# OliBus801/TARL-simulator

Measured on AMD Instinct MI355X. Metric: ppo_env_steps_per_sec, higher is better.
Workload: dtype f32; 1 GPU; mpnn+ppo train, 10000-edge torus dual graph, 16384 agents, T=256 (BASELINE config 4); envs_per_gpu=32768, parallelism=dp1, rollout_kernels=frames

## Files before the change

### tarl-simulator_amd/csrc/fused.hip

```cpp
#include "fused_common.h"

struct PlanOut {
  const int32_t* out_ptr;
  const int32_t* out_dst;
};

__global__ __launch_bounds__(FB) void k_pack_nodes(const float* __restrict__ x, Layout L, int64_t B, int64_t N,
                                                   const float* __restrict__ cong, FusedBufs fb, float4* st0_out,
                                                   PlanOut P) {
  const int64_t gid = (int64_t)blockIdx.x * FB + threadIdx.x;
  if (gid >= B * N) return;
  const int64_t i = gid / B;
  const int64_t b = gid - i * B;
  const float* xi = x + b * L.bstride + i * L.ldx;
  const int Nmax = L.Nmax;
  const float n = xi[L.col_n()];
  const int q = (int)n;
  const float tail = (q >= 1 && q <= Nmax) ? xi[q - 1] : 0.0f;
  const float head = xi[0];
  if (q < 0 || q > 127 || !(head >= 0.0f && head < 16777216.0f) || !(tail >= 0.0f && tail < 16777216.0f))
    atomicOr(fb.flags, FLAG_PACK_RANGE);
  bool dirty = q >= Nmax - 1;
  for (int sidx = q < 0 ? 0 : q; sidx < Nmax; ++sidx)
    dirty = dirty || xi[sidx] != 0.0f || xi[Nmax + sidx] != 0.0f || xi[2 * Nmax + sidx] != 0.0f;
// ... 941 lines not shown
  RowStat rs[NCH];
#pragma unroll
  for (int r = 0; r < NCH; ++r) {
    const NodeRec& nr = nodes[ri[r]];
    rs[r] = RowStat{nr.out_deg, nr.out0, nr.tt0, nr.maxn};
  }
  if (threadIdx.x == 0) s_cnt = 0;
  __syncthreads();
  float nsum = 0.0f;
  if (valid) {
    uint32_t pa[NCH], tlw[NCH], pj[NCH][4];
    uint2 hp[NCH];
    uint32_t ovf = 0u;
#pragma unroll
    for (int r = 0; r < NCH; ++r) {
      const uint32_t row = (uint32_t)ri[r] * B + b;
      pa[r] = at32<O32>(post, row);
      if (SIB) {
        if (r == 0) {
          const int32_t* od = rchunks[blockIdx.y].out4;
#pragma unroll
          for (int q = 0; q < 4; ++q) pj[0][q] = at32<O32>(post, (uint32_t)od[q] * B + b);
        } else {
#pragma unroll
          for (int q = 0; q < 4; ++q) pj[r][q] = pj[0][q];
        }
      } else {
        const int32_t* od = nodes[ri[r]].out4;
#pragma unroll
        for (int q = 0; q < 4; ++q) pj[r][q] = at32<O32>(post, (uint32_t)od[q] * B + b);
      }
    }
#pragma unroll
    for (int r = 0; r < NCH; ++r) {
      const uint32_t row = (uint32_t)ri[r] * B + b;
      hp[r] = make_uint2(0u, 0u);
      tlw[r] = 0u;
      if (Nmax < 2 || (pa[r] & (PF_ARRIVED | PF_NONEMPTY | PF_TLAUTH))) {
        hp[r] = at32<O32>(fb.hdp, row);
        tlw[r] = at32<O32>(fb.tl, row);
      }
    }
#pragma unroll
    for (int r = 0; r < NCH; ++r)
      if (live[r]) {
        bool pop;
        float n = 0.0f;
        const uint32_t i = (uint32_t)ri[r];
        const bool ev = row_phase_a<FAPI, O32>(i, b, rs[r], post, pa[r], hp[r], tlw[r], pj[r], Nmax, B, N, fb, A, t, out, &pop, &n);
        nsum += n;
        if (ev) {
          const int32_t pos = atomicAdd(&s_cnt, 1);
          if (pos < EV_CAP) {
            s_item[pos] = (uint16_t)((r << 9) | (pop ? 256 : 0) | threadIdx.x);
            s_words[pos] = make_uint4(pa[r], hp[r].x, hp[r].y, tlw[r]);
          } else {
            ovf |= (1u << r) | (pop ? (16u << r) : 0u);
          }
        }
      }
    if (ovf != 0u) {
#pragma unroll 1
      for (int r = 0; r < NCH; ++r) {
        if (!((ovf >> r) & 1u)) continue;
        uint32_t pa_r = pa[0], tl_r = tlw[0];
        uint2 hp_r = hp[0];
        int32_t i_r = ri[0];
#pragma unroll
        for (int q = 1; q < NCH; ++q) {
          pa_r = (r == q) ? pa[q] : pa_r;
          tl_r = (r == q) ? tlw[q] : tl_r;
          hp_r.x = (r == q) ? hp[q].x : hp_r.x;
          hp_r.y = (r == q) ? hp[q].y : hp_r.y;
          i_r = (r == q) ? ri[q] : i_r;
        }
        const float2 nc = row_phase_b<FAPI>((uint32_t)i_r, b, ((ovf >> (4 + r)) & 1u) != 0u, pa_r, hp_r, tl_r, nodes[i_r], out_ptr,
                                      out_dst, Nmax, B, N, fb, ag, A, a_bstride, t, out);
        nsum -= nc.y;
        if (nc.y != 0.0f) atomicAdd(&fb.acc_w[(int64_t)(blockIdx.y % (unsigned)fb.acc_slots) * B + b], nc.y);
      }
    }
  }
  const int64_t bank0 = (int64_t)(blockIdx.y % (unsigned)fb.acc_slots) * B;
  if (valid && nsum != 0.0f) atomicAdd(&fb.acc_n[bank0 + b], nsum);
  __syncthreads();
  const int32_t cnt = s_cnt < EV_CAP ? s_cnt : EV_CAP;
  for (int32_t idx = threadIdx.x; idx < cnt; idx += blockDim.x) {
    const uint32_t item = s_item[idx];
    const uint32_t r = item >> 9, lane2 = item & 255u;
    const uint4 wd = s_words[idx];
    const uint32_t b2 = blockIdx.x * blockDim.x + lane2;
    int32_t i2 = ri[0];
#pragma unroll
    for (int q = 1; q < NCH; ++q) i2 = (r == (uint32_t)q) ? ri[q] : i2;
    const float2 nc = row_phase_b<FAPI>((uint32_t)i2, b2, (item & 256u) != 0u, wd.x, make_uint2(wd.y, wd.z), wd.w, nodes[i2],
                                  out_ptr, out_dst, Nmax, B, N, fb, ag, A, a_bstride, t, out);
    if (nc.y != 0.0f) {
      atomicAdd(&fb.acc_n[bank0 + b2], -nc.y);
      atomicAdd(&fb.acc_w[bank0 + b2], nc.y);
    }
  }
}

__device__ __forceinline__ bool fused_target(const FusedBufs& fb, PlanOut P, const uint8_t* __restrict__ sel8, int64_t b,
                                             int64_t B, int64_t N, int32_t origin, int32_t* road, int32_t* cap) {
  if (origin < 0 || origin >= N) return false;
  const int64_t orow = (int64_t)origin * B + b;
  const uint32_t c = sel8[orow] & 0x7Fu;
  const long long r = (long long)(c == SEL_RAW ? fb.sel[orow] : (float)P.out_dst[P.out_ptr[origin] + (int32_t)c]);
  if (r < 0 || r >= N) return false;
  const long long room = (long long)(fb.st0[r].x - TARL_CONGESTION_FILE - (float)(fb.hdp[r * B + b].x & HD_CNT));
  *road = (int32_t)r;
  *cap = (int32_t)(room > 0x7fffffff ? 0x7fffffff : room);
  return room > 0;
}

__device__ __forceinline__ bool fused_target_words(const FusedBufs& fb, PlanOut P, const uint8_t* __restrict__ sel8,
                                                   int64_t b, int64_t B, int64_t N, int32_t origin, int32_t* road,
                                                   uint32_t* hd_out, uint32_t* tl_out) {
  if (origin < 0 || origin >= N) return false;
  const int64_t orow = (int64_t)origin * B + b;
  const uint32_t c = sel8[orow] & 0x7Fu;
  const int32_t* o4 = fb.nodes[origin].out4;
  const int32_t t0 = o4[0], t1 = o4[1], t2 = o4[2], t3 = o4[3];
  long long r;
  if (c < 4u)
    r = (long long)(float)(c == 0u ? t0 : (c == 1u ? t1 : (c == 2u ? t2 : t3)));
  else
    r = (long long)(c == SEL_RAW ? fb.sel[orow] : (float)P.out_dst[P.out_ptr[origin] + (int32_t)c]);
  if (r < 0 || r >= N) return false;
  const uint32_t hd = fb.hdp[r * B + b].x;
  *tl_out = fb.tl[r * B + b];
  const long long room = (long long)(fb.st0[r].x - TARL_CONGESTION_FILE - (float)(hd & HD_CNT));
  *road = (int32_t)r;
  *hd_out = hd;
  return room > 0;
}

struct InsLds {
  int32_t wave[INSB / 64];
  int32_t cnt, adm, lo;
  int32_t cnt2[8], adm2[8], lo2[8];
  int32_t un_agent[INS_CAP], un_road[INS_CAP], un_k[INS_CAP];
  uint32_t un_hd[INS_CAP], un_tl[INS_CAP];
};
#define s_wave L.wave
#define s_cnt L.cnt
#define s_adm L.adm
#define s_lo L.lo
#define s_un_agent L.un_agent
#define s_un_road L.un_road
#define s_un_k L.un_k
#define s_un_hd L.un_hd
#define s_un_tl L.un_tl
__device__ __forceinline__ void fused_insert_body(InsLds& L, int64_t b, int Nmax, int64_t B, int64_t N, const FusedBufs& fb, PlanOut P,
                                                  const uint8_t* __restrict__ sel8, float* __restrict__ ag, int64_t A,
                                                  int64_t a_bstride, int use_cong, float t,
                                                  int32_t* __restrict__ scratch, const float* __restrict__ entropy_in,
                                                  float* __restrict__ reward, FrameOut out,
                                                  float* __restrict__ log_prob, float* __restrict__ entropy) {
  float* agb = ag + b * a_bstride;
  int32_t* cand_agent = scratch + b * 2 * A;
  int32_t* cand_road = cand_agent + A;
  const int tid = threadIdx.x, lane = tid & 63, wid = tid >> 6;

  if (tid == 0) {
    s_cnt = 0;
    s_adm = 0;
  }
  long long lpf = 0;
  float nf = 0.0f, wf = 0.0f;
  if (wid == 0) {
    for (int64_t sl_ = lane; sl_ < fb.acc_slots; sl_ += 64) {
      lpf += fb.acc_lp[sl_ * B + b];
      nf += fb.acc_n[sl_ * B + b];
      wf += fb.acc_w[sl_ * B + b];
      fb.acc_lp[sl_ * B + b] = 0;
      fb.acc_n[sl_ * B + b] = 0.0f;
      fb.acc_w[sl_ * B + b] = 0.0f;
    }
  }
  __syncthreads();
  if (fb.a_order) {
    const int32_t* ord = fb.a_order + b * A;
    const float* dsort = fb.a_dep_sorted + b * A;
    const int32_t lo = fb.cur_lo[b];
    if (tid == 0) s_lo = 0x7fffffff;
    __syncthreads();
    for (int64_t k0 = lo; k0 < A; k0 += INSB) {
      const int64_t k = k0 + tid;
      bool notdue = false;
      if (k < A) {
        bool due, waiting;
        int32_t a, origin;
        if (fb.a_win) {
          const uint4 w = fb.a_win[b * A + k];
          waiting = fb.a_ins[b * A + k] == 0;
          due = __uint_as_float(w.x) <= t;
          origin = (int32_t)w.y;
          a = (int32_t)w.z;
        } else {
          due = dsort[k] <= t;
          a = due ? ord[k] : 0;
          waiting = due && fb.a_status[b * A + a] == 0;
          origin = waiting ? fb.a_origin[b * A + a] : 0;
        }
        notdue = !due;
        if (!due) {
          atomicMin(&s_lo, (int32_t)k);
        } else if (waiting) {
          atomicMin(&s_lo, (int32_t)k);
          int32_t road = 0, cap = 0;
          if (fb.a_win) {
            uint32_t hdw = 0u, tlw = 0u;
            if (fused_target_words(fb, P, sel8, b, B, N, origin, &road, &hdw, &tlw)) {
              const int32_t pos = atomicAdd(&s_cnt, 1);
              if (pos < INS_CAP) {
                s_un_agent[pos] = a;
                s_un_road[pos] = road;
                s_un_k[pos] = (int32_t)k;
                s_un_hd[pos] = hdw;
                s_un_tl[pos] = tlw;
              }
            }
          } else if (fused_target(fb, P, sel8, b, B, N, origin, &road, &cap)) {
            const int32_t pos = atomicAdd(&s_cnt, 1);
            if (pos < INS_CAP) {
              s_un_agent[pos] = a;
              s_un_road[pos] = road;
            }
          }
        }
      }
      if (__syncthreads_or(notdue ? 1 : 0)) break;
    }
    __syncthreads();
    if (tid == 0) fb.cur_lo[b] = s_lo == 0x7fffffff ? (int32_t)A : s_lo;
  } else {
    for (int64_t a0 = tid; a0 < A; a0 += 4 * INSB) {
      uint8_t stt[4];
      float dp[4];
  #pragma unroll
      for (int j = 0; j < 4; ++j) {
        const int64_t a = a0 + (int64_t)j * INSB;
        stt[j] = a < A ? fb.a_status[b * A + a] : (uint8_t)1;
        dp[j] = a < A ? fb.a_dep[b * A + a] : 0.0f;
      }
  #pragma unroll
      for (int j = 0; j < 4; ++j) {
        if (stt[j] == 0 && dp[j] <= t) {
          const int64_t a = a0 + (int64_t)j * INSB;
          int32_t road = 0, cap = 0;
          if (fused_target(fb, P, sel8, b, B, N, fb.a_origin[b * A + a], &road, &cap)) {
            const int32_t pos = atomicAdd(&s_cnt, 1);
            if (pos < INS_CAP) {
              s_un_agent[pos] = (int32_t)a;
              s_un_road[pos] = road;
            }
          }
        }
      }
// ... 66 lines not shown
      if (a < A && fb.a_status[b * A + a] == 0 && fb.a_dep[b * A + a] <= t)
        cnd = fused_target(fb, P, sel8, b, B, N, fb.a_origin[b * A + a], &road, &cap);
      const unsigned long long bal = __ballot(cnd);
      const int lane_off = __popcll(bal & ((1ull << lane) - 1ull));
      if (lane == 0) s_wave[wid] = __popcll(bal);
      __syncthreads();
      int32_t wbase = 0, tot = 0;
      for (int w = 0; w < INSB / 64; ++w) {
        const int32_t v = s_wave[w];
        if (w < wid) wbase += v;
        tot += v;
      }
      if (cnd) {
        cand_agent[basec + wbase + lane_off] = (int32_t)a;
        cand_road[basec + wbase + lane_off] = road;
      }
      basec += tot;
      __syncthreads();
    }
    Lc = basec;
    __threadfence_block();
    __syncthreads();
  }

  for (int32_t idx = tid; idx < Lc; idx += INSB) {
    const int32_t r = cand_road[idx];
    const int32_t a = cand_agent[idx];
    int32_t rank = 0, total = 0;
    for (int32_t k = 0; k < Lc; ++k) {
      const bool same = cand_road[k] == r;
      total += same ? 1 : 0;
      rank += (same && k < idx) ? 1 : 0;
    }
    const int64_t rrow = (int64_t)r * B + b;
    const float4 str = fb.st0[r];
    const uint32_t hd = fb.hdp[rrow].x;
    const uint32_t n0i = hd & HD_CNT;
    const float n0 = (float)n0i;
    const long long cap = (long long)(str.x - TARL_CONGESTION_FILE - n0);
    int32_t commit = 0;
    if (rank < cap) {
      const long long m = total < cap ? total : cap;
      const long long slot = (long long)n0i + rank;
      const float t_cong = use_cong ? str.w / (str.x + 10.0f - n0) : 0.0f;
      const float tt = (t_cong != t_cong) ? t_cong : fmaxf(str.y, t_cong);
      const int hoff = tl_hoff(fb.tl[rrow]);
      if (slot >= 0 && slot < Nmax) {
        slot_store(fb.slots + rrow * fb.lds + SLW * phys(hoff, (int)slot, Nmax), (float)a, t, t + tt);
      }
      agb[(int64_t)a * AG_COLS + AG_ON_WAY] = 1.0f;
      fb.a_status[b * A + a] = 1;
      if (fb.a_ins) fb.a_ins[b * A + fb.a_rank[b * A + a]] = 1;
      if (rank == 0 && n0i == 0u) {
        fb.hdp[rrow] = make_uint2(((uint32_t)a << 8) | n0i | (hd & HD_DIRTY), __float_as_uint(t + tt));
      }
      if (rank == m - 1) fb.tl[rrow] = tl_word((uint32_t)a, hoff, TLF_AUTH);
      if (rank == 0) commit = (int32_t)m;
    }
    cand_agent[idx] = commit;
  }
  __threadfence_block();
  __syncthreads();
  for (int32_t idx = tid; idx < Lc; idx += INSB) {
    const int32_t cmt = cand_agent[idx];
    if (cmt > 0) {
      const int64_t rrow = (int64_t)cand_road[idx] * B + b;
      if (out.write_gc || b < out.m_env) fb.gc8[rrow] = (uint8_t)r1_code(-1);
      const uint32_t hd = fb.hdp[rrow].x + (uint32_t)cmt;
      fb.hdp[rrow].x = hd;
      if (out.counts8) out.counts8[rrow] = (uint8_t)(hd & HD_CNT);
      if (out.countsf) out.countsf[rrow] = (float)(hd & HD_CNT);
      atomicAdd(&s_adm, cmt);
    }
  }
  __syncthreads();
  }
  if (wid == 0) {
    for (int off = 32; off > 0; off >>= 1) {
      lpf += __shfl_down(lpf, off);
      nf += __shfl_down(nf, off);
      wf += __shfl_down(wf, off);
    }
    if (lane == 0) {
      if (reward) reward[b] = -(nf + (float)s_adm);
      if (log_prob) log_prob[b] = (lpf < -(1ll << 49)) ? -INFINITY : (float)((double)lpf / LP_FIX);
      if (entropy) entropy[b] = entropy_in[0];
      if (out.leg) {
        out.leg[2 * b + 0] = s_adm;
        out.leg[2 * b + 1] = (int32_t)wf;
      }
    }
  }
}

#undef s_wave
#undef s_cnt
#undef s_adm
#undef s_lo
#undef s_un_agent
#undef s_un_road
#undef s_un_k
#undef s_un_hd
#undef s_un_tl

__global__ __launch_bounds__(INSB) void k_fused_insert(int Nmax, int64_t B, int64_t N, const FusedBufs* __restrict__ fbp, PlanOut P,
                                                       const uint8_t* __restrict__ sel8, float* __restrict__ ag,
                                                       int64_t A, int64_t a_bstride, int use_cong, float t,
                                                       int32_t* __restrict__ scratch,
                                                       const float* __restrict__ entropy_in,
                                                       float* __restrict__ reward, FrameOut out,
                                                       float* __restrict__ log_prob, float* __restrict__ entropy) {
  __shared__ InsLds L;
  fused_insert_body(L, blockIdx.x, Nmax, B, N, *fbp, P, sel8, ag, A, a_bstride, use_cong, t, scratch, entropy_in, reward,
                    out, log_prob, entropy);
}

template <int EPW>
__global__ __launch_bounds__(INSB) void k_fused_insert2(int Nmax, int64_t B, int64_t N, const FusedBufs* __restrict__ fbp, PlanOut P,
                                                        const uint8_t* __restrict__ sel8, float* __restrict__ ag,
                                                        int64_t A, int64_t a_bstride, int use_cong, float t,
                                                        int32_t* __restrict__ scratch,
                                                        const float* __restrict__ entropy_in,
                                                        float* __restrict__ reward, FrameOut out,
                                                        float* __restrict__ log_prob, float* __restrict__ entropy) {
  __shared__ InsLds L;
  const FusedBufs& fb = *fbp;
  constexpr int LPE = 64 / EPW;
  constexpr int INS_CAP2 = INS_CAP / EPW;
  const int tid = threadIdx.x, h = tid / LPE, l = tid % LPE;
  const int64_t b0 = EPW * (int64_t)blockIdx.x, b = b0 + h;
  const bool live = b < B;
  const int base = h * INS_CAP2;
  if (l == 0) {
    L.cnt2[h] = 0;
    L.adm2[h] = 0;
    L.lo2[h] = 0x7fffffff;
  }
  long long lpf = 0;
  float nf = 0.0f, wf = 0.0f;
  if (live) {
    for (int64_t sl_ = l; sl_ < fb.acc_slots; sl_ += LPE) {
      lpf += fb.acc_lp[sl_ * B + b];
      nf += fb.acc_n[sl_ * B + b];
      wf += fb.acc_w[sl_ * B + b];
    }
  }
  const int32_t lo = live ? fb.cur_lo[b] : 0;
  __syncthreads();
  bool done = !live;
  int64_t k0 = lo;
  if (live && k0 >= A) done = true;
  while (true) {
    bool notdue = false;
    if (!done) {
      const int64_t k = k0 + l;
      if (k < A) {
        const uint4 w = fb.a_win[b * A + k];
        const bool waiting = fb.a_ins[b * A + k] == 0;
        const bool due = __uint_as_float(w.x) <= t;
        const int32_t origin = (int32_t)w.y, a = (int32_t)w.z;
        notdue = !due;
        if (!due) {
          atomicMin(&L.lo2[h], (int32_t)k);
        } else if (waiting) {
          atomicMin(&L.lo2[h], (int32_t)k);
          int32_t road = 0;
          uint32_t hdw = 0u, tlw = 0u;
          if (fused_target_words(fb, P, sel8, b, B, N, origin, &road, &hdw, &tlw)) {
            const int32_t pos = atomicAdd(&L.cnt2[h], 1);
            if (pos < INS_CAP2) {
              L.un_agent[base + pos] = a;
              L.un_road[base + pos] = road;
              L.un_k[base + pos] = (int32_t)k;
              L.un_hd[base + pos] = hdw;
              L.un_tl[base + pos] = tlw;
            }
          }
        }
      }
    }
    const unsigned long long nd = __ballot(notdue);
    if (!done) {
      if (((nd >> (LPE * h)) & ((1ull << LPE) - 1ull)) != 0ull || k0 + LPE >= A)
        done = true;
      else
        k0 += LPE;
    }
    if (__ballot(!done) == 0ull) break;
  }
  __syncthreads();
  bool over = false;
#pragma unroll
  for (int e = 0; e < EPW; ++e) over = over || (L.cnt2[e] > INS_CAP2);
  if (live && l == 0) fb.cur_lo[b] = L.lo2[h] == 0x7fffffff ? (int32_t)A : L.lo2[h];
  const bool mine = live && L.cnt2[h] <= INS_CAP2;
  if (mine) {
    for (int64_t sl_ = l; sl_ < fb.acc_slots; sl_ += LPE) {
      fb.acc_lp[sl_ * B + b] = 0;
      fb.acc_n[sl_ * B + b] = 0.0f;
      fb.acc_w[sl_ * B + b] = 0.0f;
    }
    float* agb = ag + b * a_bstride;
    const int32_t Lc = L.cnt2[h];
    for (int32_t idx = l; idx < Lc; idx += LPE) {
      const int32_t r = L.un_road[base + idx];
      const int32_t a = L.un_agent[base + idx];
      int32_t rank = 0, total = 0;
      for (int32_t k = 0; k < Lc; ++k) {
        const bool same = L.un_road[base + k] == r;
        total += same ? 1 : 0;
        rank += (same && L.un_agent[base + k] < a) ? 1 : 0;
      }
      const int64_t rrow = (int64_t)r * B + b;
      const float4 str = fb.st0[r];
      const uint32_t hd = L.un_hd[base + idx];
      const uint32_t n0i = hd & HD_CNT;
      const float n0 = (float)n0i;
      const long long cap = (long long)(str.x - TARL_CONGESTION_FILE - n0);
      if (rank < cap) {
        const long long m = total < cap ? total : cap;
        const long long slot = (long long)n0i + rank;
        const float t_cong = use_cong ? str.w / (str.x + 10.0f - n0) : 0.0f;
        const float tt = (t_cong != t_cong) ? t_cong : fmaxf(str.y, t_cong);
        const int hoff = tl_hoff(L.un_tl[base + idx]);
        if (slot >= 0 && slot < Nmax) {
          slot_store(fb.slots + rrow * fb.lds + SLW * phys(hoff, (int)slot, Nmax), (float)a, t, t + tt);
        }
        agb[(int64_t)a * AG_COLS + AG_ON_WAY] = 1.0f;
        fb.a_status[b * A + a] = 1;
        fb.a_ins[b * A + L.un_k[base + idx]] = 1;
        if (rank == m - 1) fb.tl[rrow] = tl_word((uint32_t)a, hoff, TLF_AUTH);
        if (rank == 0) {
          const uint32_t cnt = n0i + (uint32_t)m;
          if (n0i == 0u) {
            fb.hdp[rrow] = make_uint2(((uint32_t)a << 8) | cnt | (hd & HD_DIRTY), __float_as_uint(t + tt));
          } else {
            fb.hdp[rrow].x = hd + (uint32_t)m;
          }
          if (out.write_gc || b < out.m_env) fb.gc8[rrow] = (uint8_t)r1_code(-1);
          if (out.counts8) out.counts8[rrow] = (uint8_t)cnt;
          if (out.countsf) out.countsf[rrow] = (float)cnt;
          atomicAdd(&L.adm2[h], (int32_t)m);
        }
      }
    }
  }
  __syncthreads();
  for (int off = LPE / 2; off > 0; off >>= 1) {
    lpf += __shfl_down(lpf, off, LPE);
    nf += __shfl_down(nf, off, LPE);
    wf += __shfl_down(wf, off, LPE);
  }
  if (mine && l == 0) {
    if (reward) reward[b] = -(nf + (float)L.adm2[h]);
    if (log_prob) log_prob[b] = (lpf < -(1ll << 49)) ? -INFINITY : (float)((double)lpf / LP_FIX);
    if (entropy) entropy[b] = entropy_in[0];
    if (out.leg) {
      out.leg[2 * b + 0] = L.adm2[h];
      out.leg[2 * b + 1] = (int32_t)wf;
    }
  }
  if (over) {
    __syncthreads();
    for (int e = 0; e < EPW; ++e) {
      if (b0 + e < B && L.cnt2[e] > INS_CAP2)
        fused_insert_body(L, b0 + e, Nmax, B, N, fb, P, sel8, ag, A, a_bstride, use_cong, t, scratch, entropy_in, reward,
                          out, log_prob, entropy);
      __syncthreads();
    }
  }
}

struct ChoiceArgs {
  const int32_t* out_ptr;
  const int32_t* out_eid;
  const int32_t* group_of_node;
  int64_t G;
  const float* thr;
  const long long* lgt;
  uint64_t pseed, pcounter;
  int nchunk, want_lp;
  uint8_t* sel_next;
  long long* acc_next;
  unsigned gx;
  unsigned choice_blocks;
};
__global__ __launch_bounds__(TILE) void k_fused_insert_choice(ChoiceArgs C, int Nmax, int64_t B, int64_t N,
                                                              const FusedBufs* __restrict__ fbp,
                                                              PlanOut P, const uint8_t* __restrict__ sel8,
                                                              float* __restrict__ ag, int64_t A, int64_t a_bstride,
                                                              int use_cong, float t, int32_t* __restrict__ scratch,
                                                              const float* __restrict__ entropy_in,
                                                              float* __restrict__ reward, FrameOut out,
                                                              float* __restrict__ log_prob,
                                                              float* __restrict__ entropy) {
  __shared__ InsLds L;
  if (blockIdx.x < (unsigned)B) {
    if (threadIdx.x >= INSB) return;
    fused_insert_body(L, (int64_t)blockIdx.x, Nmax, B, N, *fbp, P, sel8, ag, A, a_bstride, use_cong, t, scratch, entropy_in,
                      reward, out, log_prob, entropy);
  } else {
    const unsigned cb = blockIdx.x - (unsigned)B;
    fused_choice_body(cb % C.gx, cb / C.gx, C.out_ptr, C.out_eid, C.group_of_node, C.G, B, N, C.acc_next, fbp->acc_slots,
                      C.thr, C.lgt, nullptr, C.pseed, C.pcounter, C.sel_next, sel8, nullptr, C.nchunk, C.want_lp, fbp->env_base);
  }
}

FusedBufs tarl_to_bufs(const tarl_fused* f) {
  return FusedBufs{(uint2*)f->hdp,        (uint32_t*)f->tl, f->gc8,          (uint32_t*)f->post, (const float4*)f->st0,
                   f->slots,              f->ld_slots,      f->sel8,         f->sel,             (const NodeRec*)f->node_rec,
                   (const InRec*)f->in_rec, f->out_pad,
                   (long long*)f->acc_lp, f->acc_n,         f->acc_w,        f->a_origin,        f->a_dest,
                   f->a_dep,              f->a_status,      f->a_order,      f->cur_lo,          f->a_dep_sorted,
                   (const uint4*)f->a_win, f->a_ins,        f->a_rank,
                   f->acc_slots,          f->flags,         f->env_base};
}

__global__ void k_set_bufs(FusedBufs a, FusedBufs b, FusedBufs* __restrict__ dst) {
  dst[0] = a;
  dst[1] = b;
}
extern "C" int64_t tarl_fused_bufs_bytes(void) { return 2 * (int64_t)sizeof(FusedBufs); }
static int upload_bufs(const tarl_fused* f, const FusedBufs& fb, long long* acc_lp_alt, hipStream_t s, const FusedBufs** dev) {
  TARL_REQUIRE(f->bufs_dev && ((uintptr_t)f->bufs_dev) % 16 == 0, "tarl_fused.bufs_dev missing or misaligned (tarl_fused_bufs_bytes)");
  FusedBufs alt = fb;
  if (acc_lp_alt) alt.acc_lp = acc_lp_alt;
  hipLaunchKernelGGL(k_set_bufs, dim3(1), dim3(1), 0, s, fb, alt, (FusedBufs*)f->bufs_dev);
  TARL_LAUNCH_CHECK();
  *dev = (const FusedBufs*)f->bufs_dev;
  return TARL_OK;
}

static int nchunk() {
  static int v = 0;
  if (v == 0) {
    const char* e = getenv("TARL_NCHUNK");
    v = e ? atoi(e) : 4;
// ... 296 lines not shown

__global__ __launch_bounds__(FB) void k_apply_choice8(const int32_t* __restrict__ choice, const int32_t* __restrict__ out_ptr,
                                                      const int32_t* __restrict__ out_eid, int64_t B, int64_t N,
                                                      uint8_t* __restrict__ sel8) {
  const int64_t gid = (int64_t)blockIdx.x * FB + threadIdx.x;
  if (gid >= B * N) return;
  const int64_t i = gid / B, b = gid - i * B;
  const int32_t e = choice[b * N + i];
  uint32_t code = (sel8[gid] & 0x7Fu) | SEL_CARRIED;
  if (e >= 0) {
    const int32_t k0 = out_ptr[i], k1 = out_ptr[i + 1];
    for (int32_t k = k0; k < k1; ++k)
      if (out_eid[k] == e) code = (uint32_t)(k - k0);
  }
  sel8[gid] = (uint8_t)code;
}

extern "C" int tarl_fused_apply_choice(const tarl_plan* plan, const tarl_fused* f, int64_t B, const int32_t* choice,
                                       tarl_stream stream) {
  TARL_REQUIRE(plan && f && f->sel8 && choice && B >= 1, "null argument");
  if (plan->N == 0) return TARL_OK;
  hipLaunchKernelGGL(k_apply_choice8, dim3((unsigned)ceil_div(B * plan->N, FB)), dim3(FB), 0, (hipStream_t)stream, choice,
                     plan->out_ptr, plan->out_eid, B, plan->N, f->sel8);
  TARL_LAUNCH_CHECK();
  return TARL_OK;
}

#define CHOICE_CHUNK 32
#define CHOICE_FIRST 4
#define CHOICE_MAX_CHUNKS 256
struct ChoiceSide {
  hipStream_t stream;
  hipEvent_t start;
  hipEvent_t done[CHOICE_MAX_CHUNKS];
  bool ready;
};
static ChoiceSide g_choice_side[64];

static int choice_side(ChoiceSide** out) {
  int dev = 0;
  TARL_CHECK_HIP(hipGetDevice(&dev));
  ChoiceSide* cs = &g_choice_side[dev & 63];
  if (!cs->ready) {
    TARL_CHECK_HIP(hipStreamCreateWithFlags(&cs->stream, hipStreamNonBlocking));
    TARL_CHECK_HIP(hipEventCreateWithFlags(&cs->start, hipEventDisableTiming));
    for (int i = 0; i < CHOICE_MAX_CHUNKS; ++i) TARL_CHECK_HIP(hipEventCreateWithFlags(&cs->done[i], hipEventDisableTiming));
    cs->ready = true;
  }
  *out = cs;
  return TARL_OK;
}

static int insert_envs_per_wave(const tarl_fused* f, int64_t A, int64_t B, int64_t T, const float* times_host) {
  static const bool pair_ok = !(getenv("TARL_INSERT_PAIR") && atoi(getenv("TARL_INSERT_PAIR")) == 0);
  static const int epw_env = getenv("TARL_INSERT_EPW") ? atoi(getenv("TARL_INSERT_EPW")) : 0;
  int epw = A <= 20000 && B >= 12288 ? 8 : (A <= 32768 ? 4 : (A <= 65536 ? 2 : 1));
  if (f->due_rate > 0.0f) {
    const float dt = T > 1 ? times_host[1] - times_host[0] : 1.0f;
    const float per_frame = f->due_rate * (dt > 0.0f ? dt : 1.0f);
    while (epw > 1 && 2.0f * per_frame > (float)(INS_CAP / epw)) epw >>= 1;
  }
  if (epw_env == 1 || epw_env == 2 || epw_env == 4 || epw_env == 8) epw = epw_env;
  return (pair_ok && f->a_order && f->a_win) ? epw : 1;
}

static int launch_insert(int epw, hipStream_t s, int Nmax, int64_t B, int64_t N, const FusedBufs* fbt, PlanOut P,
                         const uint8_t* sel_t, float* agent_features, int64_t A, int64_t a_bstride, int use_cong, float time,
                         int32_t* ins_scratch, const float* entropy1, float* reward_t, const FrameOut& out, float* lp_t,
                         float* ent_t) {
#define INS2_LAUNCH(EPW_)                                                                                                         \
  hipLaunchKernelGGL((k_fused_insert2<EPW_>), dim3((unsigned)ceil_div(B, EPW_)), dim3(INSB), 0, s, Nmax, B, N, fbt, P, sel_t,   \
                     agent_features, A, a_bstride, use_cong, time, ins_scratch, entropy1, reward_t, out, lp_t, ent_t)
  if (epw == 8) {
    INS2_LAUNCH(8);
  } else if (epw == 4) {
    INS2_LAUNCH(4);
  } else if (epw == 2) {
    INS2_LAUNCH(2);
  } else {
    hipLaunchKernelGGL(k_fused_insert, dim3((unsigned)B), dim3(INSB), 0, s, Nmax, B, N, fbt, P, sel_t, agent_features, A,
                       a_bstride, use_cong, time, ins_scratch, entropy1, reward_t, out, lp_t, ent_t);
  }
#undef INS2_LAUNCH
  TARL_LAUNCH_CHECK();
  return TARL_OK;
}

extern "C" int64_t tarl_fused_rollout_scratch_ints(const tarl_plan* plan, int64_t T, int64_t B) {
  return plan && T >= 1 && B >= 1 ? (int64_t)(4 + 2 * FIX_CAP) + 4 * (plan->E + 4) + 2 * T * B + 16 * (plan->N + 1) : -1;
}

extern "C" int tarl_fused_rollout(const tarl_plan* plan, const tarl_fused* f, int64_t B, int32_t Nmax, int64_t T,
                                  const float* times_host, float prev_time, const float* thresholds,
                                  const int64_t* log_probs, const float* entropy1, uint64_t policy_seed,
                                  uint64_t policy_counter0, float* agent_features, int64_t A, int64_t a_bstride,
                                  const float* edge_attr, const float* log_edge_attr, float log_eps, int use_cong,
                                  uint64_t seed, uint64_t counter0, int32_t* ins_scratch, uint8_t* sel_scratch,
                                  int64_t* acc_scratch, int32_t* choice_scratch, uint8_t* choice, float* log_prob,
                                  float* entropy, float* reward,
                                  uint8_t* counts, int32_t metrics_envs, float* dtt_node, uint8_t* events, int32_t* leg,
                                  tarl_stream stream) {
  int rc = tarl_check_fused_core(plan, f, B, Nmax);
  if (rc) return rc;
  TARL_REQUIRE(T >= 1 && times_host, "bad frame count / times");
  TARL_REQUIRE(thresholds && log_probs && entropy1, "policy tables missing (call tarl_fused_policy_prepare)");
  rc = check_frame_args(plan, f, B, agent_features, A, a_bstride, ins_scratch, edge_attr, log_edge_attr);
  if (rc) return rc;
  TARL_REQUIRE(metrics_envs >= 0 && metrics_envs <= B, "metrics_envs out of range");
  TARL_REQUIRE(metrics_envs > 0 || (!dtt_node && !events), "per-node series need metrics_envs > 0");
  if (plan->N == 0) return TARL_OK;
  hipStream_t s = (hipStream_t)stream;
  const int64_t N = plan->N, NB = N * B;
  const unsigned threads = tile_threads(B);
  const dim3 grid((unsigned)ceil_div(B, threads), (unsigned)num_chunks(plan));
  const dim3 grid_c((unsigned)ceil_div(B, threads), (unsigned)ceil_div(N, nchunk_choice()));
  const dim3 grid_d((unsigned)ceil_div(B, threads), (unsigned)ceil_div(N, nchunk_dir()));
  const int want_lp = log_prob != nullptr ? 1 : 0;
  const FusedBufs fb = tarl_to_bufs(f);
  const PlanOut P{plan->out_ptr, plan->out_dst};
  auto slice = [&](int64_t t) -> uint8_t* {
    if (choice) return choice + t * NB;
    return (sel_scratch && (t & 1)) ? sel_scratch : f->sel8;
  };
  const char* knob = getenv("TARL_ROLLOUT_MERGE");
  const int mode = knob ? atoi(knob) : 2;
  const bool ahead = mode >= 2 && choice && choice_scratch && ceil_div(T, CHOICE_CHUNK) + 1 <= CHOICE_MAX_CHUNKS &&
                     ceil_div(N, CHOICE_SEG) < 65536;
  const bool merge = !ahead && mode >= 1 && (choice || sel_scratch) && acc_scratch && T > 1;
  long long* acc_buf[2] = {(long long*)f->acc_lp, merge ? (long long*)acc_scratch : (long long*)f->acc_lp};
  if (merge) TARL_CHECK_HIP(hipMemsetAsync(acc_scratch, 0, (size_t)(f->acc_slots * B) * sizeof(int64_t), s));
  const FusedBufs* fbd = nullptr;
  rc = upload_bufs(f, fb, acc_buf[1], s, &fbd);
  if (rc) return rc;
  ChoiceSide* side = nullptr;
  if (ahead) {
    rc = choice_side(&side);
    if (rc) return rc;
    int32_t* fix = choice_scratch;
    PRec* ptab = (PRec*)(choice_scratch + 4 + 2 * FIX_CAP);
    TARL_REQUIRE(((uintptr_t)ptab) % 16 == 0, "choice_scratch must be 16-byte aligned");
    TARL_CHECK_HIP(hipEventRecord(side->start, s));
    TARL_CHECK_HIP(hipStreamWaitEvent(side->stream, side->start, 0));
    TARL_CHECK_HIP(hipMemsetAsync(fix, 0, 2 * sizeof(int32_t), side->stream));
    hipLaunchKernelGGL(k_pack_ptab, dim3((unsigned)ceil_div(plan->E + 4, FB)), dim3(FB), 0, side->stream, plan->E,
                       thresholds, (const long long*)log_probs, ptab);
    TARL_LAUNCH_CHECK();
    PNode* pnode = (PNode*)(((uintptr_t)(ptab + plan->E + 4) + 63) & ~(uintptr_t)63);
    long long* lp_acc = (long long*)(pnode + N);
    hipLaunchKernelGGL(k_pack_pnode, dim3((unsigned)ceil_div(N, FB)), dim3(FB), 0, side->stream, N,
                       (const NodeRec*)f->node_rec, plan->group_of_node, thresholds, (const long long*)log_probs, pnode);
    TARL_LAUNCH_CHECK();
    for (int64_t c = 0, t0 = 0; t0 < T; ++c) {
      const int64_t want = c == 0 ? CHOICE_FIRST : CHOICE_CHUNK;
      const unsigned nf = (unsigned)(T - t0 < want ? T - t0 : want);
      static const bool quad_ok = !(getenv("TARL_CHOICE_QUAD") && atoi(getenv("TARL_CHOICE_QUAD")) == 0);
      const bool quad = quad_ok && plan->G == N && N % 4 == 0;
      hipLaunchKernelGGL(quad ? k_fused_choice_all<true> : k_fused_choice_all<false>,
                         dim3((unsigned)ceil_div(B, threads), (unsigned)ceil_div(N, CHOICE_SEG), nf),
                         dim3(threads), 0, side->stream, (const PNode*)pnode, (const PRec*)ptab,
                         plan->group_of_node, (uint32_t)plan->G, (uint32_t)B, (uint32_t)N, t0, policy_seed,
                         policy_counter0, (const uint8_t*)f->sel8, choice, log_prob ? lp_acc : nullptr, fix, f->flags,
                         (uint64_t)f->env_base);
      TARL_LAUNCH_CHECK();
      hipLaunchKernelGGL(k_choice_fixup, dim3(1), dim3(ENVB), 0, side->stream, (uint32_t)B, (uint32_t)N,
                         (const uint8_t*)f->sel8, choice, fix);
      TARL_LAUNCH_CHECK();
      if (log_prob) {
        hipLaunchKernelGGL(k_choice_lp_finish, dim3((unsigned)ceil_div((int64_t)nf * B, FB)), dim3(FB), 0, side->stream,
                           (int64_t)nf * B, lp_acc + t0 * B, log_prob + t0 * B);
        TARL_LAUNCH_CHECK();
      }
      TARL_CHECK_HIP(hipEventRecord(side->done[c], side->stream));
      t0 += nf;
    }
  } else {
    hipLaunchKernelGGL(k_fused_choice, grid_c, dim3(threads), 0, s, plan->out_ptr, plan->out_eid, plan->group_of_node,
                       plan->G, B, N, acc_buf[0], fb.acc_slots, thresholds, (const long long*)log_probs,
                       (const float*)nullptr, policy_seed, policy_counter0, slice(0), (const uint8_t*)f->sel8,
                       (int32_t*)nullptr, nchunk_choice(), want_lp, f->env_base);
    TARL_LAUNCH_CHECK();
  }
  const int epw_packed = insert_envs_per_wave(f, A, B, T, times_host);
  for (int64_t t = 0; t < T; ++t) {
    const int cur = merge ? (int)(t & 1) : 0;
    const float time = times_host[t];
    const FusedBufs* fbt = fbd + cur;
    const uint8_t* sel_t = slice(t);
    const int64_t m = metrics_envs;
    const FrameOut out{counts ? counts + t * NB : nullptr,
                       nullptr,
                       nullptr,
                       nullptr,
                       events ? events + t * N * m : nullptr,
                       dtt_node ? dtt_node + t * N * m : nullptr,
                       metrics_envs,
                       leg ? leg + t * 2 * B : nullptr,
                       t + 1 == T ? 1 : 0};
    if (ahead && (t == 0 || (t >= CHOICE_FIRST && (t - CHOICE_FIRST) % CHOICE_CHUNK == 0)))
      TARL_CHECK_HIP(hipStreamWaitEvent(s, side->done[t == 0 ? 0 : 1 + (t - CHOICE_FIRST) / CHOICE_CHUNK], 0));
    const bool timed = tarl_prof_mark(s, 0) != nullptr;
    rc = launch_direction(grid_d, threads, s, plan, f, edge_attr, log_edge_attr, sel_t, nullptr, nullptr, log_eps, time,
                          t > 0 ? times_host[t - 1] : prev_time, seed, counter0 + (uint64_t)t, B, (int)Nmax, out,
                          (counts && t > 0) ? counts + (t - 1) * NB : nullptr);
    if (rc) return rc;
    if (timed) (void)tarl_prof_mark(s, 1);
    rc = launch_rows(grid, threads, s, plan, f, fbt, (int)Nmax, B, agent_features, A, a_bstride, time, out);
    if (rc) return rc;
    if (timed) (void)tarl_prof_mark(s, 2);
    float* reward_t = reward ? reward + t * B : nullptr;
    float* lp_t = (log_prob && !ahead) ? log_prob + t * B : nullptr;
    float* ent_t = entropy ? entropy + t * B : nullptr;
    if (ahead) {
      rc = launch_insert(epw_packed, s, (int)Nmax, B, N, fbt, P, sel_t, agent_features, A, a_bstride, use_cong, time, ins_scratch,
                         entropy1, reward_t, out, lp_t, ent_t);
      if (rc) return rc;
    } else if (merge && t + 1 < T) {
      const ChoiceArgs C{plan->out_ptr, plan->out_eid, plan->group_of_node, plan->G, thresholds,
                         (const long long*)log_probs, policy_seed, policy_counter0 + (uint64_t)(t + 1), nchunk_choice(),
                         want_lp, slice(t + 1), acc_buf[cur ^ 1], grid_c.x, grid_c.x * grid_c.y};
      hipLaunchKernelGGL(k_fused_insert_choice, dim3(C.choice_blocks + (unsigned)B), dim3(threads), 0, s, C, (int)Nmax,
                         B, N, fbt, P, sel_t, agent_features, A, a_bstride, use_cong, time, ins_scratch, entropy1,
                         reward_t, out, lp_t, ent_t);
      TARL_LAUNCH_CHECK();
    } else {
      hipLaunchKernelGGL(k_fused_insert, dim3((unsigned)B), dim3(INSB), 0, s, (int)Nmax, B, N, fbt, P, sel_t,
                         agent_features, A, a_bstride, use_cong, time, ins_scratch, entropy1, reward_t, out, lp_t, ent_t);
      TARL_LAUNCH_CHECK();
      if (t + 1 < T) {
        hipLaunchKernelGGL(k_fused_choice, grid_c, dim3(threads), 0, s, plan->out_ptr, plan->out_eid,
                           plan->group_of_node, plan->G, B, N, acc_buf[cur], fb.acc_slots, thresholds,
                           (const long long*)log_probs, (const float*)nullptr, policy_seed,
                           policy_counter0 + (uint64_t)(t + 1), slice(t + 1), sel_t, (int32_t*)nullptr, nchunk_choice(),
                           want_lp, f->env_base);
        TARL_LAUNCH_CHECK();
      }
    }
    if (timed) (void)tarl_prof_mark(s, 3);
  }
  if (slice(T - 1) != f->sel8)
    TARL_CHECK_HIP(hipMemcpyAsync(f->sel8, slice(T - 1), (size_t)NB, hipMemcpyDeviceToDevice, s));
  return TARL_OK;
}

__global__ __launch_bounds__(FB) void k_obs_keep(const float4* __restrict__ obs, int64_t row4,
                                                 const int32_t* __restrict__ env, const int32_t* __restrict__ slot,
                                                 float4* __restrict__ keep) {
  const int64_t j = (int64_t)blockIdx.x * FB + threadIdx.x;
  if (j >= row4) return;
  keep[(int64_t)slot[blockIdx.y] * row4 + j] = obs[(int64_t)env[blockIdx.y] * row4 + j];
}

__global__ __launch_bounds__(256) void k_sel8_from_choice8(uint8_t* __restrict__ choice8, uint8_t* __restrict__ sel8,
                                                           int64_t B, int64_t N) {
  __shared__ uint8_t tile[64][68];
  const int lane = threadIdx.x & 63, w = threadIdx.x >> 6;
  const int64_t b0 = (int64_t)blockIdx.x * 64, i0 = (int64_t)blockIdx.y * 64;
#pragma unroll 4
  for (int r = w; r < 64; r += 4) {
    const int64_t b = b0 + r, i = i0 + lane;
    tile[r][lane] = (b < B && i < N) ? choice8[b * N + i] : (uint8_t)0;
  }
  __syncthreads();
#pragma unroll 4
  for (int r = w; r < 64; r += 4) {
    const int64_t i = i0 + r, b = b0 + lane;
    if (b < B && i < N) {
      uint32_t c = tile[lane][r];
      if (c & SEL_CARRIED) {
        c = (sel8[i * B + b] & 0x7Fu) | SEL_CARRIED;
        choice8[b * N + i] = (uint8_t)c;
      }
      sel8[i * B + b] = (uint8_t)c;
    }
  }
}

extern "C" int tarl_fused_set_actions(const tarl_plan* plan, const tarl_fused* f, int64_t B, uint8_t* choice8,
                                      tarl_stream stream) {
  TARL_REQUIRE(plan && f && f->sel8 && choice8, "null argument");
  TARL_REQUIRE(B >= 1, "bad batch size");
  if (plan->N == 0) return TARL_OK;
  hipLaunchKernelGGL(k_sel8_from_choice8, dim3((unsigned)ceil_div(B, 64), (unsigned)ceil_div(plan->N, 64)), dim3(256), 0,
                     (hipStream_t)stream, choice8, f->sel8, B, plan->N);
  TARL_LAUNCH_CHECK();
  return TARL_OK;
}

extern "C" int tarl_fused_rollout_policy(const tarl_plan* plan, const tarl_fused* f, int64_t B, int32_t Nmax, int64_t T,
                                         const float* times_host, float prev_time, const float* x, int64_t x_bstride,
                                         int64_t ldx, float* agent_features, int64_t A, int64_t a_bstride,
                                         const float* edge_attr, const float* log_edge_attr, float log_eps, int use_cong,
                                         const float* w1, const float* b1, const float* w2, const float* b2,
                                         const float* w3, const float* b3, int precision, float temperature,
                                         uint64_t policy_seed, uint64_t policy_counter0, uint64_t seed,
                                         uint64_t counter0, const int64_t* keep_ptr_host, const int32_t* keep_env,
                                         const int32_t* keep_slot, float* obs_keep, float* obs_scratch,
                                         float* logits_scratch, void* dist_scratch, int32_t* ins_scratch,
                                         uint8_t* choice8, float* log_prob, float* reward, uint8_t* counts,
                                         int32_t metrics_envs, float* dtt_node, uint8_t* events, int32_t* leg,
                                         tarl_stream stream) {
  int rc = tarl_check_fused_core(plan, f, B, Nmax);
  if (rc) return rc;
  TARL_REQUIRE(T >= 1 && times_host, "bad frame count / times");
  TARL_REQUIRE(x && obs_scratch && logits_scratch && dist_scratch, "observation / logits / sampler scratch missing");
  TARL_REQUIRE(!keep_ptr_host || (keep_env && keep_slot && obs_keep), "keep list without its arrays");
  TARL_REQUIRE(precision >= 0 && precision <= 2,
               "precision: 0 = fp32 MFMA logits, 1 = bf16 logits on bf16 observations, 2 = fp32-accurate logits on the bf16 pipe (bf16x3)");
  rc = check_frame_args(plan, f, B, agent_features, A, a_bstride, ins_scratch, edge_attr, log_edge_attr);
  if (rc) return rc;
  TARL_REQUIRE(metrics_envs >= 0 && metrics_envs <= B, "metrics_envs out of range");
  TARL_REQUIRE(metrics_envs > 0 || (!dtt_node && !events), "per-node series need metrics_envs > 0");
  if (plan->N == 0) return TARL_OK;
  hipStream_t s = (hipStream_t)stream;
  const int64_t N = plan->N, NB = N * B;
  const unsigned threads = tile_threads(B);
  const dim3 grid((unsigned)ceil_div(B, threads), (unsigned)num_chunks(plan));
  const dim3 grid_d((unsigned)ceil_div(B, threads), (unsigned)ceil_div(N, nchunk_dir()));
  const FusedBufs fbh = tarl_to_bufs(f);
  const FusedBufs* fb = nullptr;
  rc = upload_bufs(f, fbh, nullptr, s, &fb);
// ... 91 lines not shown
```

### tarl-simulator_amd/csrc/fused_common.h

```cpp
#pragma once

#include <float.h>
#include <math.h>
#include <stdlib.h>

#include "tarl_common.h"

#define FB 256
#define ENVB 1024
#define TILE 256
#define LOG_EPS_P 1e-8f
#define INS_CAP 192
#define INSB 64

#define HD_DIRTY 0x80u
#define HD_CNT 0x7Fu
#define TLF_AUTH 1u
#define PF_ARRIVED 1u
#define PF_NONEMPTY 2u
#define PF_TLAUTH 4u
#define SEL_RAW 0x7Fu
#define SEL_CARRIED 0x80u
#define INRANK_NONE 0xFEu
#define FLAG_COUNT_AT_NMAX 1
#define FLAG_AMBIGUOUS_EDGES 2
#define FLAG_PACK_RANGE 4
#define FLAG_CHOICE_OVERFLOW 8

struct __attribute__((aligned(4))) InRec {
  int32_t src;
  int32_t rank;
  float ea;
  float max_src;
  int32_t eid;
};
struct __attribute__((aligned(16))) NodeRec {
  int32_t in0, in_deg;
  int32_t out0, out_deg;
  float maxn, ff, road, cong;
  float tt0;
  int32_t pad_[3];
  int32_t out4[4];
  InRec in4[4];
};
#define NODE_REC_WORDS 36
#define IN_REC_WORDS 5
static_assert(sizeof(NodeRec) == NODE_REC_WORDS * 4 && sizeof(InRec) == IN_REC_WORDS * 4, "record sizes are part of the buffer contract (tarl_hip/ops.py: FusedState)");

struct FusedBufs {
  uint2* hdp;
  uint32_t* tl;
  uint8_t* gc8;
  uint32_t* post;
  const float4* st0;
  float* slots;
  int64_t lds;
  uint8_t* sel8;
  float* sel;
  const NodeRec* nodes;
  const InRec* in_rec;
  const int32_t* out_pad;
  long long* acc_lp;
  float* acc_n;
  float* acc_w;
  int32_t* a_origin;
  int32_t* a_dest;
  float* a_dep;
  uint8_t* a_status;
  const int32_t* a_order;
  int32_t* cur_lo;
  const float* a_dep_sorted;
  const uint4* a_win;
  uint8_t* a_ins;
  const int32_t* a_rank;
  int64_t acc_slots;
  int32_t* flags;
  int64_t env_base;
};

struct FrameOut {
  uint8_t* counts8;
  float* countsf;
  uint8_t* popped;
  uint8_t* withdrawn;
  uint8_t* events;
  float* dtt_node;
  int32_t m_env;
  int32_t* leg;
  int32_t write_gc;
};

#define LP_FIX 4294967296.0

#ifndef TARL_SLW
#define TARL_SLW 3
#endif
#define SLW TARL_SLW
#define SLW_ALIGN (SLW == 8 ? 8 : 1)
__device__ __forceinline__ void slot_store(float* w, float id, float arr, float dep) {
#if TARL_SLW == 8
  reinterpret_cast<float4*>(w)[0] = make_float4(id, arr, dep, 0.0f);
  reinterpret_cast<float4*>(w)[1] = make_float4(0.0f, 0.0f, 0.0f, 0.0f);
#else
  w[0] = id;
  w[1] = arr;
  w[2] = dep;
#endif
}
struct SlotRec {
  float id, arr, dep;
};
__device__ __forceinline__ SlotRec slot_load(const float* r) {
#if TARL_SLW == 8
  const float4 v = *reinterpret_cast<const float4*>(r);
  return SlotRec{v.x, v.y, v.z};
#else
  return SlotRec{r[0], r[1], r[2]};
#endif
}
__device__ __forceinline__ uint32_t r1_code(int g) { return (uint32_t)(g + 1); }
__device__ __forceinline__ int r1_g(uint32_t code) { return (int)code - 1; }
__device__ __forceinline__ int tl_hoff(uint32_t tlw) { return (int)((tlw >> 1) & 127u); }
__device__ __forceinline__ uint32_t tl_word(uint32_t tail_id, int hoff, uint32_t auth) {
  return (tail_id << 8) | ((uint32_t)hoff << 1) | auth;
}
__device__ __forceinline__ int pending_g(uint32_t tlw, int n, uint32_t code, int Nmax) {
  return (tlw & TLF_AUTH) ? r1_g(code) : (n < Nmax - 1 ? n : -1);
}
__device__ __forceinline__ int phys(int hoff, int s, int Nmax) {
  int p = hoff + s;
  return p >= Nmax ? p - Nmax : p;
}
__device__ __forceinline__ float head_arrival(const float* __restrict__ slots, int64_t lds, const uint8_t* __restrict__ gc8,
                                              int64_t row, uint32_t hd, uint32_t tlw, int Nmax, float t_last) {
  if ((hd & HD_CNT) == 0u) {
    if (pending_g(tlw, 0, (uint32_t)gc8[row], Nmax) >= 0) return t_last;
    if (!(hd & HD_DIRTY)) return 0.0f;
  }
  return slots[row * lds + SLW * tl_hoff(tlw) + 1];
}

__device__ __forceinline__ float sel_value(const FusedBufs& fb, const int32_t* __restrict__ out_ptr,
                                           const int32_t* __restrict__ out_dst, int64_t i, int64_t row) {
  const uint32_t c = fb.sel8[row] & 0x7Fu;
  return c == SEL_RAW ? fb.sel[row] : (float)out_dst[out_ptr[i] + (int32_t)c];
}
__device__ __forceinline__ float entry_tt(const float4 st, float n) {
  const float t_cong = st.w / (st.x + 10.0f - n);
  return (t_cong != t_cong) ? t_cong : fmaxf(st.y, t_cong);
}

FusedBufs tarl_to_bufs(const tarl_fused* f);
int tarl_check_fused_core(const tarl_plan* plan, const tarl_fused* f, int64_t B, int32_t Nmax);
int tarl_fused_dead_slots(const tarl_plan* plan, const tarl_fused* f, int64_t B, int32_t Nmax, int materialise,
                          tarl_stream stream);
hipEvent_t tarl_prof_mark(hipStream_t s, int tag);
int tarl_graphdist_rollout_at(const tarl_plan* plan, const float* logits, int64_t B, float temperature,
                              const float* uniform, uint64_t seed, uint64_t counter, void* scratch, int32_t* choice,
                              uint8_t* choice8, uint8_t* sel8, float* log_prob, int64_t env_base, tarl_stream stream);
```

Baseline: 40.88 million env-steps/s.

## Compute per-frame reward from stored counts in one batched count-sum kernel

When per-frame counts and rewards are both requested, the per-step atomic accumulation of node occupancy into acc_n is skipped. The reward is recomputed after the rollout by a new kernel that sums the uint8 counts over nodes for every frame and environment, using packed byte arithmetic and nontemporal vector loads. The insert kernels also skip loading and clearing accumulator banks whose results are not needed. This trades many scattered atomics and accumulator traffic for one extra streaming pass over the T×N×B counts array. It relies on the reward equalling the negative total count, and an env var restores the old atomic path.

Result: no change. 41.02 million env-steps/s (median of 3 runs) (+0.4%).

```diff
diff --git a/tarl-simulator_amd/csrc/fused.hip b/tarl-simulator_amd/csrc/fused.hip
--- a/tarl-simulator_amd/csrc/fused.hip
+++ b/tarl-simulator_amd/csrc/fused.hip
@@ -1047,7 +1047,7 @@
     }
   }
   const int64_t bank0 = (int64_t)(blockIdx.y % (unsigned)fb.acc_slots) * B;
-  if (valid && nsum != 0.0f) atomicAdd(&fb.acc_n[bank0 + b], nsum);
+  if (valid && nsum != 0.0f && !out.sum_later) atomicAdd(&fb.acc_n[bank0 + b], nsum);
   __syncthreads();
   const int32_t cnt = s_cnt < EV_CAP ? s_cnt : EV_CAP;
   for (int32_t idx = threadIdx.x; idx < cnt; idx += blockDim.x) {
@@ -1061,7 +1061,7 @@
     const float2 nc = row_phase_b<FAPI>((uint32_t)i2, b2, (item & 256u) != 0u, wd.x, make_uint2(wd.y, wd.z), wd.w, nodes[i2],
                                   out_ptr, out_dst, Nmax, B, N, fb, ag, A, a_bstride, t, out);
     if (nc.y != 0.0f) {
-      atomicAdd(&fb.acc_n[bank0 + b2], -nc.y);
+      if (!out.sum_later) atomicAdd(&fb.acc_n[bank0 + b2], -nc.y);
       atomicAdd(&fb.acc_w[bank0 + b2], nc.y);
     }
   }
@@ -1133,15 +1133,16 @@
     s_cnt = 0;
     s_adm = 0;
   }
+  const bool need_lp = log_prob != nullptr, need_n = !out.sum_later, need_w = out.leg != nullptr;
   long long lpf = 0;
   float nf = 0.0f, wf = 0.0f;
   if (wid == 0) {
     for (int64_t sl_ = lane; sl_ < fb.acc_slots; sl_ += 64) {
-      lpf += fb.acc_lp[sl_ * B + b];
-      nf += fb.acc_n[sl_ * B + b];
-      wf += fb.acc_w[sl_ * B + b];
-      fb.acc_lp[sl_ * B + b] = 0;
-      fb.acc_n[sl_ * B + b] = 0.0f;
+      if (need_lp) lpf += fb.acc_lp[sl_ * B + b];
+      if (need_n) nf += fb.acc_n[sl_ * B + b];
+      if (need_w) wf += fb.acc_w[sl_ * B + b];
+      if (need_lp) fb.acc_lp[sl_ * B + b] = 0;
+      if (need_n) fb.acc_n[sl_ * B + b] = 0.0f;
       fb.acc_w[sl_ * B + b] = 0.0f;
     }
   }
@@ -1374,7 +1375,7 @@
       wf += __shfl_down(wf, off);
     }
     if (lane == 0) {
-      if (reward) reward[b] = -(nf + (float)s_adm);
+      if (reward && need_n) reward[b] = -(nf + (float)s_adm);
       if (log_prob) log_prob[b] = (lpf < -(1ll << 49)) ? -INFINITY : (float)((double)lpf / LP_FIX);
       if (entropy) entropy[b] = entropy_in[0];
       if (out.leg) {
@@ -1428,13 +1429,14 @@
     L.adm2[h] = 0;
     L.lo2[h] = 0x7fffffff;
   }
+  const bool need_lp = log_prob != nullptr, need_n = !out.sum_later, need_w = out.leg != nullptr;
   long long lpf = 0;
   float nf = 0.0f, wf = 0.0f;
   if (live) {
     for (int64_t sl_ = l; sl_ < fb.acc_slots; sl_ += LPE) {
-      lpf += fb.acc_lp[sl_ * B + b];
-      nf += fb.acc_n[sl_ * B + b];
-      wf += fb.acc_w[sl_ * B + b];
+      if (need_lp) lpf += fb.acc_lp[sl_ * B + b];
+      if (need_n) nf += fb.acc_n[sl_ * B + b];
+      if (need_w) wf += fb.acc_w[sl_ * B + b];
     }
   }
   const int32_t lo = live ? fb.cur_lo[b] : 0;
@@ -1488,8 +1490,8 @@
   const bool mine = live && L.cnt2[h] <= INS_CAP2;
   if (mine) {
     for (int64_t sl_ = l; sl_ < fb.acc_slots; sl_ += LPE) {
-      fb.acc_lp[sl_ * B + b] = 0;
-      fb.acc_n[sl_ * B + b] = 0.0f;
+      if (need_lp) fb.acc_lp[sl_ * B + b] = 0;
+      if (need_n) fb.acc_n[sl_ * B + b] = 0.0f;
       fb.acc_w[sl_ * B + b] = 0.0f;
     }
     float* agb = ag + b * a_bstride;
@@ -1544,7 +1546,7 @@
     wf += __shfl_down(wf, off, LPE);
   }
   if (mine && l == 0) {
-    if (reward) reward[b] = -(nf + (float)L.adm2[h]);
+    if (reward && need_n) reward[b] = -(nf + (float)L.adm2[h]);
     if (log_prob) log_prob[b] = (lpf < -(1ll << 49)) ? -INFINITY : (float)((double)lpf / LP_FIX);
     if (entropy) entropy[b] = entropy_in[0];
     if (out.leg) {
@@ -2007,6 +2009,89 @@
                        a_bstride, use_cong, time, ins_scratch, entropy1, reward_t, out, lp_t, ent_t);
   }
 #undef INS2_LAUNCH
+  TARL_LAUNCH_CHECK();
+  return TARL_OK;
+}
+
+#define CS_WAVES 4
+#define CS_UNROLL 8
+typedef uint32_t cs_u32x4 __attribute__((ext_vector_type(4)));
+template <int W>
+__global__ __launch_bounds__(64 * CS_WAVES) void k_count_sum(const uint8_t* __restrict__ counts, int64_t B, int64_t N,
+                                                             unsigned gx, float* __restrict__ reward) {
+  __shared__ uint32_t s_sum[CS_WAVES][W][64];
+  const unsigned lane = threadIdx.x & 63u, y = threadIdx.x >> 6;
+  const int64_t t = blockIdx.x / gx;
+  const int64_t b0 = (int64_t)(blockIdx.x % gx) * (64 * W);
+  const int64_t bl = b0 + (int64_t)lane * W;
+  const uint8_t* src = counts + t * N * B + bl;
+  uint32_t sum[W];
+#pragma unroll
+  for (int j = 0; j < W; ++j) sum[j] = 0u;
+  if (bl < B) {
+    if constexpr (W == 16) {
+      for (int64_t n0 = y; n0 < N; n0 += (int64_t)CS_WAVES * 256) {
+        uint32_t ev[4] = {0u, 0u, 0u, 0u}, od[4] = {0u, 0u, 0u, 0u};
+        const int64_t n1 = n0 + (int64_t)CS_WAVES * 256 < N ? n0 + (int64_t)CS_WAVES * 256 : N;
+        for (int64_t n = n0; n < n1; n += (int64_t)CS_WAVES * CS_UNROLL) {
+          cs_u32x4 v[CS_UNROLL];
+#pragma unroll
+          for (int u = 0; u < CS_UNROLL; ++u) {
+            const int64_t nu = n + (int64_t)u * CS_WAVES;
+            v[u] = cs_u32x4{0u, 0u, 0u, 0u};
+            if (nu < n1) v[u] = __builtin_nontemporal_load(reinterpret_cast<const cs_u32x4*>(src + nu * B));
+          }
+#pragma unroll
+          for (int u = 0; u < CS_UNROLL; ++u) {
+            const uint32_t w[4] = {v[u].x, v[u].y, v[u].z, v[u].w};
+#pragma unroll
+            for (int k = 0; k < 4; ++k) {
+              ev[k] += w[k] & 0x00FF00FFu;
+              od[k] += (w[k] >> 8) & 0x00FF00FFu;
+            }
+          }
+        }
+#pragma unroll
+        for (int k = 0; k < 4; ++k) {
+          sum[4 * k + 0] += ev[k] & 0xFFFFu;
+          sum[4 * k + 1] += od[k] & 0xFFFFu;
+          sum[4 * k + 2] += ev[k] >> 16;
+          sum[4 * k + 3] += od[k] >> 16;
+        }
+      }
+    } else {
+      for (int64_t n = y; n < N; n += (int64_t)CS_WAVES * CS_UNROLL) {
+        uint32_t v[CS_UNROLL];
+#pragma unroll
+        for (int u = 0; u < CS_UNROLL; ++u) {
+          const int64_t nu = n + (int64_t)u * CS_WAVES;
+          v[u] = nu < N ? (uint32_t)__builtin_nontemporal_load(src + nu * B) : 0u;
+        }
+#pragma unroll
+        for (int u = 0; u < CS_UNROLL; ++u) sum[0] += v[u];
+      }
+    }
+  }
+#pragma unroll
+  for (int j = 0; j < W; ++j) s_sum[y][j][lane] = sum[j];
+  __syncthreads();
+  for (unsigned e = threadIdx.x; e < 64u * W; e += 64u * CS_WAVES) {
+    const unsigned ln = e / W, j = e % W;
+    uint32_t tot = 0u;
+#pragma unroll
+    for (int w = 0; w < CS_WAVES; ++w) tot += s_sum[w][j][ln];
+    if (b0 + e < B) reward[t * B + b0 + e] = -(float)tot;
+  }
+}
+
+static int launch_count_sum(hipStream_t s, const uint8_t* counts, int64_t T, int64_t N, int64_t B, float* reward) {
+  const bool vec = B % 16 == 0 && ((uintptr_t)counts) % 16 == 0;
+  const int64_t gx = ceil_div(B, vec ? 64 * 16 : 64);
+  TARL_REQUIRE(T * gx < ((int64_t)1 << 31), "too many frames x environments for one count-sum launch");
+  if (vec)
+    hipLaunchKernelGGL(k_count_sum<16>, dim3((unsigned)(T * gx)), dim3(64 * CS_WAVES), 0, s, counts, B, N, (unsigned)gx, reward);
+  else
+    hipLaunchKernelGGL(k_count_sum<1>, dim3((unsigned)(T * gx)), dim3(64 * CS_WAVES), 0, s, counts, B, N, (unsigned)gx, reward);
   TARL_LAUNCH_CHECK();
   return TARL_OK;
 }
@@ -2106,6 +2191,8 @@
     TARL_LAUNCH_CHECK();
   }
   const int epw_packed = insert_envs_per_wave(f, A, B, T, times_host);
+  const char* cs_knob = getenv("TARL_COUNT_SUM");
+  const bool sum_later = counts && reward && !(cs_knob && strcmp(cs_knob, "atomic") == 0);
   for (int64_t t = 0; t < T; ++t) {
     const int cur = merge ? (int)(t & 1) : 0;
     const float time = times_host[t];
@@ -2120,7 +2207,8 @@
                        dtt_node ? dtt_node + t * N * m : nullptr,
                        metrics_envs,
                        leg ? leg + t * 2 * B : nullptr,
-                       t + 1 == T ? 1 : 0};
+                       t + 1 == T ? 1 : 0,
+                       sum_later ? 1 : 0};
     if (ahead && (t == 0 || (t >= CHOICE_FIRST && (t - CHOICE_FIRST) % CHOICE_CHUNK == 0)))
       TARL_CHECK_HIP(hipStreamWaitEvent(s, side->done[t == 0 ? 0 : 1 + (t - CHOICE_FIRST) / CHOICE_CHUNK], 0));
     const bool timed = tarl_prof_mark(s, 0) != nullptr;
@@ -2132,7 +2220,7 @@
     rc = launch_rows(grid, threads, s, plan, f, fbt, (int)Nmax, B, agent_features, A, a_bstride, time, out);
     if (rc) return rc;
     if (timed) (void)tarl_prof_mark(s, 2);
-    float* reward_t = reward ? reward + t * B : nullptr;
+    float* reward_t = (reward && !sum_later) ? reward + t * B : nullptr;
     float* lp_t = (log_prob && !ahead) ? log_prob + t * B : nullptr;
     float* ent_t = entropy ? entropy + t * B : nullptr;
     if (ahead) {
@@ -2161,6 +2249,10 @@
       }
     }
     if (timed) (void)tarl_prof_mark(s, 3);
+  }
+  if (sum_later) {
+    rc = launch_count_sum(s, counts, T, N, B, reward);
+    if (rc) return rc;
   }
   if (slice(T - 1) != f->sel8)
     TARL_CHECK_HIP(hipMemcpyAsync(f->sel8, slice(T - 1), (size_t)NB, hipMemcpyDeviceToDevice, s));
diff --git a/tarl-simulator_amd/csrc/fused_common.h b/tarl-simulator_amd/csrc/fused_common.h
--- a/tarl-simulator_amd/csrc/fused_common.h
+++ b/tarl-simulator_amd/csrc/fused_common.h
@@ -3,6 +3,7 @@
 #include <float.h>
 #include <math.h>
 #include <stdlib.h>
+#include <string.h>
 
 #include "tarl_common.h"
 
@@ -88,6 +89,7 @@
   int32_t m_env;
   int32_t* leg;
   int32_t write_gc;
+  int32_t sum_later;
 };
 
 #define LP_FIX 4294967296.0
```
